# HpWang-whu/RoReg

Hardware: AMD Instinct MI355X
Metric: pair-registrations/sec (higher is better)
Workload: dtype f32 (every f32 operand enters the fp16 matrix cores as hi + lo fp16 under a per-keypoint power-of-two block scale: <= 22 significant bits relative to a CONSERVATIVE per-keypoint bound -- measured on the extractor: the bound sits 2^2..2^6 above the keypoint's true coefficient maximum (config.f16x2_sc

## Files before the change

### roreg_amd/csrc/mfma_match.hip

```cpp
#include "common.h"
#include "primitives.h"

#pragma clang fp contract(off)

namespace {

struct MatchTask {
    const float *desc0, *desc1;
    const int64_t *rows0, *rows1;
    int32_t m0, m1;
};

constexpr int F = 32, TILE = 128, LP = 36;
constexpr float PAD_NORM = 1e30f;

struct WS {
    float *G;
    float *N;
    unsigned *AM;
    unsigned long long *PK;
    unsigned *MX;
};
__host__ __device__ inline size_t ws_task_bytes(int P) { return (size_t)2 * P * (F * 4 + 4 + 4 + 8) + 64; }
__device__ __forceinline__ WS ws_of(char *base, int task, int P) {
    char *p = base + (size_t)task * ws_task_bytes(P);
    WS w;
    w.PK = reinterpret_cast<unsigned long long *>(p); p += (size_t)2 * P * 8;
    w.G = reinterpret_cast<float *>(p); p += (size_t)2 * P * F * 4;
    w.N = reinterpret_cast<float *>(p); p += (size_t)2 * P * 4;
    w.AM = reinterpret_cast<unsigned *>(p); p += (size_t)2 * P * 4;
    w.MX = reinterpret_cast<unsigned *>(p);
    return w;
}

__device__ __forceinline__ unsigned f2o(float x) { const unsigned b = __float_as_uint(x); return b ^ ((b >> 31) ? 0xffffffffu : 0x80000000u); }
__device__ __forceinline__ float o2f(unsigned k) { return __uint_as_float(k ^ ((k >> 31) ? 0x80000000u : 0xffffffffu)); }

__global__ __launch_bounds__(256) void mm_prepare_kernel(const MatchTask *__restrict__ tasks, int P, char *__restrict__ wsb) {
    const int task = blockIdx.z >> 1, side = blockIdx.z & 1;
    const MatchTask t = tasks[task];
    const WS w = ws_of(wsb, task, P);
    const float *desc = side ? t.desc1 : t.desc0;
    const int64_t *rows = side ? t.rows1 : t.rows0;
    const int m = side ? t.m1 : t.m0;
    const int j = blockIdx.x * 8 + (threadIdx.x >> 5), f = threadIdx.x & 31;
    if (blockIdx.x == 0 && threadIdx.x == 0) w.MX[side] = 0u;
    if (j >= P) return;
    float v = 0.f;
    if (j < m) v = desc[(size_t)(rows ? rows[j] : (int64_t)j) * F + f];
    w.G[((size_t)side * P + j) * F + f] = v;
    float s = v * v;
#pragma unroll
    for (int o = 16; o > 0; o >>= 1) s += __shfl_xor(s, o);
    if (f == 0) {
        w.N[(size_t)side * P + j] = j < m ? s : PAD_NORM;
        w.AM[(size_t)side * P + j] = 0xffffffffu;
        w.PK[(size_t)side * P + j] = ~0ull;
    }
}

__global__ __launch_bounds__(256) void mm_maxnorm_kernel(const MatchTask *__restrict__ tasks, int P, char *__restrict__ wsb) {
    const int task = blockIdx.z >> 1, side = blockIdx.z & 1;
    const MatchTask t = tasks[task];
    const WS w = ws_of(wsb, task, P);
    const int m = side ? t.m1 : t.m0;
    const int j = blockIdx.x * 256 + threadIdx.x;
    float v = (j < m) ? w.N[(size_t)side * P + j] : 0.f;
#pragma unroll
    for (int o = 32; o > 0; o >>= 1) v = fmaxf(v, __shfl_xor(v, o));
    if ((threadIdx.x & 63) == 0 && v > 0.f) atomicMax(&w.MX[side], __float_as_uint(v));
}

__device__ __forceinline__ f32x16 mfma6(const bf16x8 (&a)[3], const bf16x8 (&b)[3], f32x16 c) {
    c = __builtin_amdgcn_mfma_f32_32x32x16_bf16(a[2], b[0], c, 0, 0, 0);
    c = __builtin_amdgcn_mfma_f32_32x32x16_bf16(a[1], b[1], c, 0, 0, 0);
    c = __builtin_amdgcn_mfma_f32_32x32x16_bf16(a[0], b[2], c, 0, 0, 0);
    c = __builtin_amdgcn_mfma_f32_32x32x16_bf16(a[1], b[0], c, 0, 0, 0);
    c = __builtin_amdgcn_mfma_f32_32x32x16_bf16(a[0], b[1], c, 0, 0, 0);
    c = __builtin_amdgcn_mfma_f32_32x32x16_bf16(a[0], b[0], c, 0, 0, 0);
    return c;
}

__device__ __forceinline__ int norm_exp(float n2) {
    if (!(n2 > 0.f) || !(n2 < __builtin_inff())) return 0;
    int ex;
    (void)frexpf(n2, &ex);
    return 14 - ((ex + 1) >> 1);
}
__device__ __forceinline__ f32x16 mfma3(const f16x8 (&a)[2], const f16x8 (&b)[2], f32x16 c) {
    c = __builtin_amdgcn_mfma_f32_32x32x16_f16(a[1], b[0], c, 0, 0, 0);
    c = __builtin_amdgcn_mfma_f32_32x32x16_f16(a[0], b[1], c, 0, 0, 0);
    c = __builtin_amdgcn_mfma_f32_32x32x16_f16(a[0], b[0], c, 0, 0, 0);
    return c;
}

__device__ __forceinline__ float exact_dist(const float *__restrict__ s, const float *__restrict__ t) {
    float acc = 0.f;
#pragma unroll
    for (int f = 0; f < F; ++f) {
        const float d = __fsub_rn(s[f], t[f]);
        acc = __fadd_rn(acc, __fmul_rn(d, d));
    }
    return sqrtf(__fadd_rn(acc, 1e-7f));
}

template <bool VERIFY, int NP >
__global__ __launch_bounds__(256, 2) void mm_tile_kernel(const MatchTask *__restrict__ tasks, int P, char *__restrict__ wsb) {
    __shared__ __attribute__((aligned(16))) float S[TILE * LP], T[TILE * LP];
    __shared__ float n0s[TILE], n1s[TILE], thr0[TILE], thr1[TILE];
    __shared__ float xs0[TILE], xs1[TILE], is0[TILE], is1[TILE];
    const int task = blockIdx.z;
    const MatchTask t = tasks[task];
    const int i0 = blockIdx.y * TILE, j0 = blockIdx.x * TILE;
    if (i0 >= t.m0 || j0 >= t.m1) return;
    const WS w = ws_of(wsb, task, P);
    const int tid = threadIdx.x, lane = tid & 63, wv = tid >> 6;
    const int wm = wv & 1, wn = wv >> 1, jl = lane & 31, h = lane >> 5;

    {
        const float4 *g0 = reinterpret_cast<const float4 *>(w.G + (size_t)i0 * F);
        const float4 *g1 = reinterpret_cast<const float4 *>(w.G + ((size_t)P + j0) * F);
        for (int q = tid; q < TILE * F / 4; q += 256) {
            const int r = q >> 3, c4 = q & 7;
            *reinterpret_cast<float4 *>(S + r * LP + c4 * 4) = g0[q];
            *reinterpret_cast<float4 *>(T + r * LP + c4 * 4) = g1[q];
        }
        if (tid < TILE) {
            const float a = w.N[i0 + tid], b = w.N[(size_t)P + j0 + tid];
            n0s[tid] = a; n1s[tid] = b;
            const int ea = NP == 2 ? norm_exp(a) : 0, eb = NP == 2 ? norm_exp(b) : 0;
            xs0[tid] = ldexpf(1.f, ea); is0[tid] = ldexpf(1.f, -ea); xs1[tid] = ldexpf(1.f, eb); is1[tid] = ldexpf(1.f, -eb);
            if (VERIFY) {
                const float mx0 = __uint_as_float(w.MX[0]), mx1 = __uint_as_float(w.MX[1]);
                thr0[tid] = o2f(w.AM[i0 + tid]) + (1e-4f * (a + mx1) + 1e-6f);
                thr1[tid] = o2f(w.AM[(size_t)P + j0 + tid]) + (1e-4f * (b + mx0) + 1e-6f);
            }
        }
    }
    __syncthreads();

    f32x16 c[2][2], ct[2][2];
#pragma unroll
    for (int a = 0; a < 2; ++a)
#pragma unroll
        for (int b = 0; b < 2; ++b)
#pragma unroll
            for (int r = 0; r < 16; ++r) { c[a][b][r] = 0.f; ct[a][b][r] = 0.f; }
#pragma unroll
    for (int st = 0; st < 2; ++st) {
        using frag = typename std::conditional<NP == 3, bf16x8, f16x8>::type;
        frag sf[2][NP], tf[2][NP];
#pragma unroll
        for (int g = 0; g < 2; ++g) {
            float x8[8];
            const int rs = wm * 64 + g * 32 + jl, rt = wn * 64 + g * 32 + jl;
            const float4 *ps = reinterpret_cast<const float4 *>(S + rs * LP + st * 16 + h * 8);
            const float4 u0 = ps[0], u1 = ps[1];
            x8[0] = u0.x; x8[1] = u0.y; x8[2] = u0.z; x8[3] = u0.w; x8[4] = u1.x; x8[5] = u1.y; x8[6] = u1.z; x8[7] = u1.w;
            if constexpr (NP == 3) split3(x8, sf[g][0], sf[g][1], sf[g][2]); else split2(x8, xs0[rs], sf[g][0], sf[g][1]);
            const float4 *pt = reinterpret_cast<const float4 *>(T + rt * LP + st * 16 + h * 8);
            const float4 v0 = pt[0], v1 = pt[1];
            x8[0] = v0.x; x8[1] = v0.y; x8[2] = v0.z; x8[3] = v0.w; x8[4] = v1.x; x8[5] = v1.y; x8[6] = v1.z; x8[7] = v1.w;
            if constexpr (NP == 3) split3(x8, tf[g][0], tf[g][1], tf[g][2]); else split2(x8, xs1[rt], tf[g][0], tf[g][1]);
        }
#pragma unroll
        for (int a = 0; a < 2; ++a)
#pragma unroll
            for (int b = 0; b < 2; ++b) {
                if constexpr (NP == 3) {
                    c[a][b] = mfma6(sf[a], tf[b], c[a][b]);
                    if (!VERIFY) ct[a][b] = mfma6(tf[a], sf[b], ct[a][b]);
                } else {
                    c[a][b] = mfma3(sf[a], tf[b], c[a][b]);
                    if (!VERIFY) ct[a][b] = mfma3(tf[a], sf[b], ct[a][b]);
                }
            }
    }
#define DOT_C(a, b, r, ir, jc) (NP == 2 ? (c[a][b][r] * is0[ir]) * is1[jc] : c[a][b][r])
#define DOT_CT(a, b, r, jr, ic) (NP == 2 ? (ct[a][b][r] * is1[jr]) * is0[ic] : ct[a][b][r])

    if (!VERIFY) {
#pragma unroll
        for (int b = 0; b < 2; ++b) {
            const int jc = wn * 64 + b * 32 + jl;
            const float nj = n1s[jc];
            float mn = __builtin_inff();
#pragma unroll
            for (int a = 0; a < 2; ++a)
#pragma unroll
                for (int r = 0; r < 16; ++r) {
                    const int ir = wm * 64 + a * 32 + (r & 3) + 8 * (r >> 2) + 4 * h;
                    mn = fminf(mn, (n0s[ir] + nj) - 2.f * DOT_C(a, b, r, ir, jc));
                }
            mn = fminf(mn, __shfl_xor(mn, 32));
            if (h == 0 && j0 + jc < t.m1) atomicMin(&w.AM[(size_t)P + j0 + jc], f2o(mn));
        }
#pragma unroll
        for (int b = 0; b < 2; ++b) {
            const int ic = wm * 64 + b * 32 + jl;
            const float ni = n0s[ic];
            float mn = __builtin_inff();
#pragma unroll
            for (int a = 0; a < 2; ++a)
#pragma unroll
                for (int r = 0; r < 16; ++r) {
                    const int jr = wn * 64 + a * 32 + (r & 3) + 8 * (r >> 2) + 4 * h;
                    mn = fminf(mn, (ni + n1s[jr]) - 2.f * DOT_CT(a, b, r, jr, ic));
                }
            mn = fminf(mn, __shfl_xor(mn, 32));
            if (h == 0 && i0 + ic < t.m0) atomicMin(&w.AM[i0 + ic], f2o(mn));
        }
    } else {
#pragma unroll
        for (int b = 0; b < 2; ++b) {
            const int jc = wn * 64 + b * 32 + jl;
            const float nj = n1s[jc], tj = thr1[jc];
#pragma unroll
            for (int a = 0; a < 2; ++a)
#pragma unroll
                for (int r = 0; r < 16; ++r) {
                    const int ir = wm * 64 + a * 32 + (r & 3) + 8 * (r >> 2) + 4 * h;
                    const float av = (n0s[ir] + nj) - 2.f * DOT_C(a, b, r, ir, jc);
                    const bool k0 = av <= thr0[ir], k1 = av <= tj;
                    if (k0 || k1) {
                        const float d = exact_dist(S + ir * LP, T + jc * LP);
                        const unsigned long long db = (unsigned long long)__float_as_uint(d) << 32;
                        if (k0 && j0 + jc < t.m1) atomicMin(&w.PK[i0 + ir], db | (unsigned)(j0 + jc));
                        if (k1 && i0 + ir < t.m0) atomicMin(&w.PK[(size_t)P + j0 + jc], db | (unsigned)(i0 + ir));
                    }
                }
        }
    }
#undef DOT_C
#undef DOT_CT
}

constexpr int TP = TILE * F;
__device__ __forceinline__ int swz_piece(int row, int c) { return row * 8 + (c ^ ((row >> 1) & 7)); }
__device__ __forceinline__ float exact_dist_swz(const float *__restrict__ s_tile, int ir, const float *__restrict__ t_tile, int jc) {
    float acc = 0.f;
#pragma unroll
    for (int f = 0; f < F; ++f) {
        const float sv = s_tile[swz_piece(ir, f >> 2) * 4 + (f & 3)], tv = t_tile[swz_piece(jc, f >> 2) * 4 + (f & 3)];
        const float d = __fsub_rn(sv, tv);
        acc = __fadd_rn(acc, __fmul_rn(d, d));
    }
    return sqrtf(__fadd_rn(acc, 1e-7f));
}

template <bool VERIFY>
__global__ __launch_bounds__(256, 2) void mm_strip_kernel(const MatchTask *__restrict__ tasks, int P, char *__restrict__ wsb) {
    extern __shared__ __attribute__((aligned(16))) char smem[];
    float *S = reinterpret_cast<float *>(smem);
    float *Tb = S + TP;
    float *n0s = Tb + 2 * TP, *xs0 = n0s + TILE, *is0 = xs0 + TILE, *thr0 = is0 + TILE;
    float *n1s = thr0 + TILE, *xs1 = n1s + 2 * TILE, *is1 = xs1 + 2 * TILE, *thr1 = is1 + 2 * TILE;
    unsigned *cm = reinterpret_cast<unsigned *>(thr1 + 2 * TILE);
    const int task = blockIdx.y;
    const MatchTask t = tasks[task];
    const int i0 = blockIdx.x * TILE;
    if (i0 >= t.m0 || t.m1 <= 0) return;
    const WS w = ws_of(wsb, task, P);
    const int tid = threadIdx.x, lane = tid & 63, wv = tid >> 6;
    const int wm = wv & 1, wn = wv >> 1, jl = lane & 31, h = lane >> 5;
    const int ntj = (t.m1 + TILE - 1) / TILE;
    const float mx0 = VERIFY ? __uint_as_float(w.MX[0]) : 0.f, mx1 = VERIFY ? __uint_as_float(w.MX[1]) : 0.f;

    auto dma_tile = [&](const float *src, float *dst) {
#pragma unroll
        for (int k = 0; k < 4; ++k) {
            const int q = k * 256 + tid, row = q >> 3, cs = q & 7;
            __builtin_amdgcn_global_load_lds((const __attribute__((address_space(1))) void *)(src + swz_piece(row, cs) * 4),
                                             (__attribute__((address_space(3))) void *)(dst + (k * 256 + wv * 64) * 4), 16, 0, 0);
        }
    };
    auto load_consts = [&](int jt) -> float {
        const int r = tid & (TILE - 1);
        if (tid < TILE) return w.N[(size_t)P + jt * TILE + r];
        return VERIFY ? o2f(w.AM[(size_t)P + jt * TILE + r]) : 0.f;
    };
    auto store_consts = [&](int buf, float v) {
        const int r = tid & (TILE - 1);
        if (tid < TILE) {
            const int e = norm_exp(v);
            n1s[buf * TILE + r] = v; xs1[buf * TILE + r] = ldexpf(1.f, e); is1[buf * TILE + r] = ldexpf(1.f, -e);
        } else if (VERIFY) thr1[buf * TILE + r] = v;
    };

    dma_tile(w.G + (size_t)i0 * F, S);
    dma_tile(w.G + (size_t)P * F, Tb);
    {
        const float c0 = load_consts(0);
        if (tid < TILE) {
            const float a = w.N[i0 + tid];
            const int e = norm_exp(a);
            n0s[tid] = a; xs0[tid] = ldexpf(1.f, e); is0[tid] = ldexpf(1.f, -e);
            if (VERIFY) thr0[tid] = o2f(w.AM[i0 + tid]) + (1e-4f * (a + mx1) + 1e-6f);
        }
        store_consts(0, c0);
        if (!VERIFY)
            for (int j = tid; j < P; j += 256) cm[j] = 0xffffffffu;
    }
    asm volatile("s_waitcnt vmcnt(0) lgkmcnt(0)" ::: "memory");
    __syncthreads();

    f16x8 sf[2][2][2];
#pragma unroll
    for (int st = 0; st < 2; ++st)
#pragma unroll
        for (int g = 0; g < 2; ++g) {
            const int rs = wm * 64 + g * 32 + jl;
            const float4 u0 = *reinterpret_cast<const float4 *>(S + swz_piece(rs, st * 4 + h * 2) * 4);
            const float4 u1 = *reinterpret_cast<const float4 *>(S + swz_piece(rs, st * 4 + h * 2 + 1) * 4);
            const float x8[8] = {u0.x, u0.y, u0.z, u0.w, u1.x, u1.y, u1.z, u1.w};
            split2(x8, xs0[rs], sf[st][g][0], sf[st][g][1]);
        }
    f32x16 rmin[2];
#pragma unroll
    for (int a = 0; a < 2; ++a)
#pragma unroll
        for (int r = 0; r < 16; ++r) rmin[a][r] = __builtin_inff();

    for (int jt = 0; jt < ntj; ++jt) {
        const int buf = jt & 1, j0 = jt * TILE;
        const float *T = Tb + buf * TP;
        float cnext = 0.f;
        if (jt + 1 < ntj) {
            dma_tile(w.G + ((size_t)P + j0 + TILE) * F, Tb + (buf ^ 1) * TP);
            cnext = load_consts(jt + 1);
        }
        f32x16 c[2][2];
#pragma unroll
        for (int a = 0; a < 2; ++a)
#pragma unroll
            for (int b = 0; b < 2; ++b)
#pragma unroll
                for (int r = 0; r < 16; ++r) c[a][b][r] = 0.f;
#pragma unroll
        for (int st = 0; st < 2; ++st) {
            f16x8 tf[2][2];
#pragma unroll
            for (int g = 0; g < 2; ++g) {
                const int rt = wn * 64 + g * 32 + jl;
                const float4 v0 = *reinterpret_cast<const float4 *>(T + swz_piece(rt, st * 4 + h * 2) * 4);
                const float4 v1 = *reinterpret_cast<const float4 *>(T + swz_piece(rt, st * 4 + h * 2 + 1) * 4);
                const float x8[8] = {v0.x, v0.y, v0.z, v0.w, v1.x, v1.y, v1.z, v1.w};
                split2(x8, xs1[buf * TILE + rt], tf[g][0], tf[g][1]);
            }
#pragma unroll
            for (int a = 0; a < 2; ++a)
#pragma unroll
                for (int b = 0; b < 2; ++b) c[a][b] = mfma3(sf[st][a], tf[b], c[a][b]);
        }
#pragma unroll
        for (int b = 0; b < 2; ++b) {
            const int jc = wn * 64 + b * 32 + jl;
            const float nj = n1s[buf * TILE + jc], isj = is1[buf * TILE + jc];
            if constexpr (!VERIFY) {
                float mn = __builtin_inff();
#pragma unroll
                for (int a = 0; a < 2; ++a)
#pragma unroll
                    for (int r = 0; r < 16; ++r) {
                        const int ir = wm * 64 + a * 32 + (r & 3) + 8 * (r >> 2) + 4 * h;
                        const float av = (n0s[ir] + nj) - 2.f * ((c[a][b][r] * is0[ir]) * isj);
                        mn = fminf(mn, av);
                        rmin[a][r] = fminf(rmin[a][r], av);
                    }
                mn = fminf(mn, __shfl_xor(mn, 32));
                if (h == 0) atomicMin(cm + j0 + jc, f2o(mn));
            } else {
                const float tj = thr1[buf * TILE + jc] + (1e-4f * (nj + mx0) + 1e-6f);
                unsigned m0 = 0u, m1 = 0u;
#pragma unroll
                for (int a = 0; a < 2; ++a)
#pragma unroll
                    for (int r = 0; r < 16; ++r) {
                        const int ir = wm * 64 + a * 32 + (r & 3) + 8 * (r >> 2) + 4 * h;
                        const float av = (n0s[ir] + nj) - 2.f * ((c[a][b][r] * is0[ir]) * isj);
                        m0 |= (av <= thr0[ir] ? 1u : 0u) << (a * 16 + r);
                        m1 |= (av <= tj ? 1u : 0u) << (a * 16 + r);
                    }
                unsigned m = m0 | m1;
                while (m) {
                    const int q = __ffs(m) - 1;
                    m &= m - 1;
                    const int ir = wm * 64 + (q >> 4) * 32 + (q & 3) + 8 * ((q & 15) >> 2) + 4 * h;
                    const float d = exact_dist_swz(S, ir, T, jc);
                    const unsigned long long db = (unsigned long long)__float_as_uint(d) << 32;
                    if (((m0 >> q) & 1u) && j0 + jc < t.m1) atomicMin(&w.PK[i0 + ir], db | (unsigned)(j0 + jc));
                    if (((m1 >> q) & 1u) && i0 + ir < t.m0) atomicMin(&w.PK[(size_t)P + j0 + jc], db | (unsigned)(i0 + ir));
                }
            }
        }
        if (jt + 1 < ntj) store_consts(buf ^ 1, cnext);
        asm volatile("s_waitcnt vmcnt(0) lgkmcnt(0)" ::: "memory");
        __syncthreads();
    }
    if constexpr (!VERIFY) {
#pragma unroll
        for (int a = 0; a < 2; ++a)
#pragma unroll
            for (int r = 0; r < 16; ++r) {
                float v = rmin[a][r];
#pragma unroll
                for (int o = 16; o > 0; o >>= 1) v = fminf(v, __shfl_xor(v, o));
                const int ir = wm * 64 + a * 32 + (r & 3) + 8 * (r >> 2) + 4 * h;
                if (jl == 0 && i0 + ir < t.m0) atomicMin(&w.AM[i0 + ir], f2o(v));
            }
        for (int j = tid; j < t.m1; j += 256) atomicMin(&w.AM[(size_t)P + j], cm[j]);
    }
}

__global__ __launch_bounds__(1024) void mm_mutual_kernel(const MatchTask *__restrict__ tasks, int P, char *__restrict__ wsb, int out_pitch,
                                                         int64_t *__restrict__ match_all, int32_t *__restrict__ counts) {
    __shared__ int wave_cnt[16];
    __shared__ int base;
    const int task = blockIdx.x;
    const MatchTask t = tasks[task];
    const WS w = ws_of(wsb, task, P);
    const unsigned long long *p01 = w.PK, *p10 = w.PK + P;
    int64_t *match_out = match_all + (size_t)task * out_pitch * 2;
    const int m = t.m1 > 0 ? t.m0 : 0;
    const int tid = threadIdx.x, lane = tid & 63, wv = tid >> 6;
    if (tid == 0) base = 0;
    __syncthreads();
    for (int start = 0; start < m; start += 1024) {
        const int i = start + tid;
        bool keep = false;
        int64_t j = 0;
        if (i < m) {
            j = (int64_t)(p01[i] & 0xffffffffu);
            keep = j < (int64_t)t.m1 && (int64_t)(p10[j] & 0xffffffffu) == (int64_t)i;
        }
        const unsigned long long mask = __ballot(keep);
        const int before = __popcll(mask & ((1ull << lane) - 1ull));
        if (lane == 0) wave_cnt[wv] = __popcll(mask);
        __syncthreads();
        int woff = 0, total = 0;
#pragma unroll
        for (int q = 0; q < 16; ++q) {
            const int cq = wave_cnt[q];
            if (q < wv) woff += cq;
            total += cq;
        }
        const int b0 = base;
        if (keep) {
            const int pos = b0 + woff + before;
            match_out[2 * pos] = t.rows0 ? t.rows0[i] : (int64_t)i;
            match_out[2 * pos + 1] = t.rows1 ? t.rows1[j] : j;
        }
        __syncthreads();
        if (tid == 0) base = b0 + total;
        __syncthreads();
    }
    if (tid == 0) counts[task] = base;
}

}

extern "C" size_t roreg_mutual_match_batch_workspace(int n_tasks, int max_m) {
    const int P = (max_m + TILE - 1) / TILE * TILE;
    return (size_t)n_tasks * ws_task_bytes(P > 0 ? P : TILE);
}

extern "C" int roreg_mutual_match_batch(const roreg_match_task *tasks_dev, int n_tasks, int max_m, int64_t *match_out, int32_t *counts_out,
                                        void *workspace, size_t workspace_bytes, void *stream) {
    if (n_tasks == 0) return 0;
    ROREG_REQUIRE(tasks_dev && match_out && counts_out && workspace && n_tasks > 0 && max_m >= 0, "roreg_mutual_match_batch: bad arguments");
    ROREG_REQUIRE(workspace_bytes >= roreg_mutual_match_batch_workspace(n_tasks, max_m), "roreg_mutual_match_batch: workspace too small");
    ROREG_REQUIRE(n_tasks <= 65535, "roreg_mutual_match_batch: too many tasks in one call (%d)", n_tasks);
    static_assert(sizeof(roreg_match_task) == sizeof(MatchTask), "roreg_match_task layout");
    hipStream_t s = roreg::as_stream(stream);
    const MatchTask *tasks = reinterpret_cast<const MatchTask *>(tasks_dev);
    const int P = max_m > 0 ? (max_m + TILE - 1) / TILE * TILE : TILE;
    char *ws = reinterpret_cast<char *>(workspace);
    const int out_pitch = (max_m + 1) & ~1;
    if (max_m > 0) {
        hipLaunchKernelGGL(mm_prepare_kernel, dim3(P / 8, 1, 2 * n_tasks), dim3(256), 0, s, tasks, P, ws);
        hipLaunchKernelGGL(mm_maxnorm_kernel, dim3(P / 256 + 1, 1, 2 * n_tasks), dim3(256), 0, s, tasks, P, ws);
        const dim3 grid(P / TILE, P / TILE, n_tasks);
        roreg::ProfScope prof(roreg::PROF_MM_TILE, s);
        static const bool bf16x3 = [] { const char *e = getenv("ROREG_MATCH_BF16X3"); return e && e[0] == '1'; }();
        static const bool tiles = [] { const char *e = getenv("ROREG_MATCH_TILES"); return e && e[0] == '1'; }();
        const size_t lds_strip = (size_t)(3 * TP + 12 * TILE) * 4 + (size_t)P * 4;
        if (!bf16x3 && !tiles && lds_strip <= 80 * 1024) {
            const dim3 sgrid(P / TILE, n_tasks);
            auto ka = mm_strip_kernel<false>; auto kb = mm_strip_kernel<true>;
            hipError_t e1 = hipFuncSetAttribute(reinterpret_cast<const void *>(ka), hipFuncAttributeMaxDynamicSharedMemorySize, (int)lds_strip);
            hipError_t e2 = hipFuncSetAttribute(reinterpret_cast<const void *>(kb), hipFuncAttributeMaxDynamicSharedMemorySize, (int)lds_strip);
            if (e1 != hipSuccess || e2 != hipSuccess) { roreg::set_error("roreg_mutual_match_batch: hipFuncSetAttribute(%zu) failed", lds_strip); return 1; }
            hipLaunchKernelGGL(ka, sgrid, dim3(256), lds_strip, s, tasks, P, ws);
            hipLaunchKernelGGL(kb, sgrid, dim3(256), lds_strip, s, tasks, P, ws);
        } else if (bf16x3) {
            hipLaunchKernelGGL((mm_tile_kernel<false, 3>), grid, dim3(256), 0, s, tasks, P, ws);
            hipLaunchKernelGGL((mm_tile_kernel<true, 3>), grid, dim3(256), 0, s, tasks, P, ws);
        } else {
            hipLaunchKernelGGL((mm_tile_kernel<false, 2>), grid, dim3(256), 0, s, tasks, P, ws);
            hipLaunchKernelGGL((mm_tile_kernel<true, 2>), grid, dim3(256), 0, s, tasks, P, ws);
        }
    }
    hipLaunchKernelGGL(mm_mutual_kernel, dim3(n_tasks), dim3(1024), 0, s, tasks, P, ws, out_pitch, match_out, counts_out);
    ROREG_CHECK_LAUNCH("roreg_mutual_match_batch");
    return 0;
}
```

Before: 1063.

## Precompute fp16 hi/lo splits, triple-buffer tiles, queue exact-distance checks in LDS

The prepare kernel now computes the scaled fp16 hi/lo split of each descriptor once and stores it in a new workspace buffer. The strip kernel DMAs these fp16 tiles straight into a three-slot LDS ring, prefetching two tiles ahead with a partial vmcnt wait. This removes the per-tile split work and the per-tile norm-constant setup. In the verify pass, candidate pairs are pushed into an LDS queue and the exact distances are computed later from global fp32 rows, instead of immediately from the swizzled LDS tiles. That evens out warp divergence but adds workspace memory, global reads during the drain, and more complex synchronisation.

```diff
diff --git a/roreg_amd/csrc/mfma_match.hip b/roreg_amd/csrc/mfma_match.hip
--- a/roreg_amd/csrc/mfma_match.hip
+++ b/roreg_amd/csrc/mfma_match.hip
@@ -16,17 +16,19 @@
 
 struct WS {
     float *G;
+    _Float16 *H;
     float *N;
     unsigned *AM;
     unsigned long long *PK;
     unsigned *MX;
 };
-__host__ __device__ inline size_t ws_task_bytes(int P) { return (size_t)2 * P * (F * 4 + 4 + 4 + 8) + 64; }
+__host__ __device__ inline size_t ws_task_bytes(int P) { return (size_t)2 * P * (F * 4 + F * 4 + 4 + 4 + 8) + 64; }
 __device__ __forceinline__ WS ws_of(char *base, int task, int P) {
     char *p = base + (size_t)task * ws_task_bytes(P);
     WS w;
     w.PK = reinterpret_cast<unsigned long long *>(p); p += (size_t)2 * P * 8;
     w.G = reinterpret_cast<float *>(p); p += (size_t)2 * P * F * 4;
+    w.H = reinterpret_cast<_Float16 *>(p); p += (size_t)2 * P * F * 4;
     w.N = reinterpret_cast<float *>(p); p += (size_t)2 * P * 4;
     w.AM = reinterpret_cast<unsigned *>(p); p += (size_t)2 * P * 4;
     w.MX = reinterpret_cast<unsigned *>(p);
@@ -35,6 +37,13 @@
 
 __device__ __forceinline__ unsigned f2o(float x) { const unsigned b = __float_as_uint(x); return b ^ ((b >> 31) ? 0xffffffffu : 0x80000000u); }
 __device__ __forceinline__ float o2f(unsigned k) { return __uint_as_float(k ^ ((k >> 31) ? 0x80000000u : 0xffffffffu)); }
+
+__device__ __forceinline__ int norm_exp(float n2) {
+    if (!(n2 > 0.f) || !(n2 < __builtin_inff())) return 0;
+    int ex;
+    (void)frexpf(n2, &ex);
+    return 14 - ((ex + 1) >> 1);
+}
 
 __global__ __launch_bounds__(256) void mm_prepare_kernel(const MatchTask *__restrict__ tasks, int P, char *__restrict__ wsb) {
     const int task = blockIdx.z >> 1, side = blockIdx.z & 1;
@@ -52,8 +61,19 @@
     float s = v * v;
 #pragma unroll
     for (int o = 16; o > 0; o >>= 1) s += __shfl_xor(s, o);
+    const float nrm = j < m ? s : PAD_NORM;
+    float x8[8];
+#pragma unroll
+    for (int e = 0; e < 8; ++e) x8[e] = __shfl(v, (f & 3) * 8 + e, 32);
+    if (f < 4) {
+        f16x8 hi, lo;
+        split2(x8, ldexpf(1.f, norm_exp(nrm)), hi, lo);
+        _Float16 *hrow = w.H + ((size_t)side * P + j) * (2 * F);
+        *reinterpret_cast<f16x8 *>(hrow + f * 8) = hi;
+        *reinterpret_cast<f16x8 *>(hrow + F + f * 8) = lo;
+    }
     if (f == 0) {
-        w.N[(size_t)side * P + j] = j < m ? s : PAD_NORM;
+        w.N[(size_t)side * P + j] = nrm;
         w.AM[(size_t)side * P + j] = 0xffffffffu;
         w.PK[(size_t)side * P + j] = ~0ull;
     }
@@ -81,12 +101,6 @@
     return c;
 }
 
-__device__ __forceinline__ int norm_exp(float n2) {
-    if (!(n2 > 0.f) || !(n2 < __builtin_inff())) return 0;
-    int ex;
-    (void)frexpf(n2, &ex);
-    return 14 - ((ex + 1) >> 1);
-}
 __device__ __forceinline__ f32x16 mfma3(const f16x8 (&a)[2], const f16x8 (&b)[2], f32x16 c) {
     c = __builtin_amdgcn_mfma_f32_32x32x16_f16(a[1], b[0], c, 0, 0, 0);
     c = __builtin_amdgcn_mfma_f32_32x32x16_f16(a[0], b[1], c, 0, 0, 0);
@@ -237,70 +251,96 @@
 
 constexpr int TP = TILE * F;
 __device__ __forceinline__ int swz_piece(int row, int c) { return row * 8 + (c ^ ((row >> 1) & 7)); }
-__device__ __forceinline__ float exact_dist_swz(const float *__restrict__ s_tile, int ir, const float *__restrict__ t_tile, int jc) {
+
+__device__ __forceinline__ unsigned lds_addr(const void *p) { return (unsigned)(size_t)(const __attribute__((address_space(3))) void *)p; }
+__device__ __forceinline__ void lds_umin(unsigned addr, unsigned v) { asm volatile("ds_min_u32 %0, %1" ::"v"(addr), "v"(v) : "memory"); }
+__device__ __forceinline__ void lds_store(unsigned addr, unsigned v) { asm volatile("ds_write_b32 %0, %1" ::"v"(addr), "v"(v) : "memory"); }
+__device__ __forceinline__ unsigned lds_add_rtn(unsigned addr, unsigned v) {
+    unsigned r;
+    asm volatile("ds_add_rtn_u32 %0, %1, %2\n\ts_waitcnt lgkmcnt(0)" : "=v"(r) : "v"(addr), "v"(v) : "memory");
+    return r;
+}
+
+__device__ __forceinline__ void exact_update(const WS &w, const MatchTask &t, int P, int i, int j, bool k0, bool k1) {
+    const float4 *ps = reinterpret_cast<const float4 *>(w.G + (size_t)i * F);
+    const float4 *pt = reinterpret_cast<const float4 *>(w.G + ((size_t)P + j) * F);
     float acc = 0.f;
 #pragma unroll
-    for (int f = 0; f < F; ++f) {
-        const float sv = s_tile[swz_piece(ir, f >> 2) * 4 + (f & 3)], tv = t_tile[swz_piece(jc, f >> 2) * 4 + (f & 3)];
-        const float d = __fsub_rn(sv, tv);
-        acc = __fadd_rn(acc, __fmul_rn(d, d));
-    }
-    return sqrtf(__fadd_rn(acc, 1e-7f));
+    for (int q0 = 0; q0 < F / 4; q0 += 2) {
+        const float4 u[2] = {ps[q0], ps[q0 + 1]}, v[2] = {pt[q0], pt[q0 + 1]};
+#pragma unroll
+        for (int q = 0; q < 2; ++q) {
+            const float sv[4] = {u[q].x, u[q].y, u[q].z, u[q].w}, tv[4] = {v[q].x, v[q].y, v[q].z, v[q].w};
+#pragma unroll
+            for (int f = 0; f < 4; ++f) {
+                const float d = __fsub_rn(sv[f], tv[f]);
+                acc = __fadd_rn(acc, __fmul_rn(d, d));
+            }
+        }
+    }
+    const float d = sqrtf(__fadd_rn(acc, 1e-7f));
+    const unsigned long long db = (unsigned long long)__float_as_uint(d) << 32;
+    if (k0 && j < t.m1) atomicMin(&w.PK[i], db | (unsigned)j);
+    if (k1 && i < t.m0) atomicMin(&w.PK[(size_t)P + j], db | (unsigned)i);
 }
 
 template <bool VERIFY>
 __global__ __launch_bounds__(256, 2) void mm_strip_kernel(const MatchTask *__restrict__ tasks, int P, char *__restrict__ wsb) {
     extern __shared__ __attribute__((aligned(16))) char smem[];
-    float *S = reinterpret_cast<float *>(smem);
-    float *Tb = S + TP;
-    float *n0s = Tb + 2 * TP, *xs0 = n0s + TILE, *is0 = xs0 + TILE, *thr0 = is0 + TILE;
-    float *n1s = thr0 + TILE, *xs1 = n1s + 2 * TILE, *is1 = xs1 + 2 * TILE, *thr1 = is1 + 2 * TILE;
-    unsigned *cm = reinterpret_cast<unsigned *>(thr1 + 2 * TILE);
+    char *ring = smem;
+    float *n0s = reinterpret_cast<float *>(ring + 3 * TP * 4), *k0s = n0s + TILE, *thr0 = k0s + TILE;
+    float *n1s = thr0 + TILE;
+    unsigned *am1 = reinterpret_cast<unsigned *>(n1s + 3 * TILE);
+    unsigned *cm = am1 + 3 * TILE;
+    unsigned *qctl = cm;
+    unsigned *queue = cm + 4;
+    const unsigned QCAP = (unsigned)P + 3 * TILE - 4;
     const int task = blockIdx.y;
     const MatchTask t = tasks[task];
     const int i0 = blockIdx.x * TILE;
     if (i0 >= t.m0 || t.m1 <= 0) return;
     const WS w = ws_of(wsb, task, P);
-    const int tid = threadIdx.x, lane = tid & 63, wv = tid >> 6;
+    const int tid = threadIdx.x, lane = tid & 63, wv = __builtin_amdgcn_readfirstlane(tid >> 6);
     const int wm = wv & 1, wn = wv >> 1, jl = lane & 31, h = lane >> 5;
     const int ntj = (t.m1 + TILE - 1) / TILE;
     const float mx0 = VERIFY ? __uint_as_float(w.MX[0]) : 0.f, mx1 = VERIFY ? __uint_as_float(w.MX[1]) : 0.f;
-
-    auto dma_tile = [&](const float *src, float *dst) {
-#pragma unroll
-        for (int k = 0; k < 4; ++k) {
-            const int q = k * 256 + tid, row = q >> 3, cs = q & 7;
-            __builtin_amdgcn_global_load_lds((const __attribute__((address_space(1))) void *)(src + swz_piece(row, cs) * 4),
-                                             (__attribute__((address_space(3))) void *)(dst + (k * 256 + wv * 64) * 4), 16, 0, 0);
-        }
+    const char *H0 = reinterpret_cast<const char *>(w.H), *H1 = H0 + (size_t)P * (4 * F);
+
+    const unsigned piece0 = (unsigned)swz_piece(tid >> 3, tid & 7) * 16u;
+    auto dma_rows = [&](const char *src, char *dst) {
+#pragma unroll
+        for (int k = 0; k < 4; ++k)
+            __builtin_amdgcn_global_load_lds((const __attribute__((address_space(1))) void *)(src + k * 4096 + (size_t)piece0),
+                                             (__attribute__((address_space(3))) void *)(dst + (k * 256 + wv * 64) * 16), 16, 0, 0);
     };
-    auto load_consts = [&](int jt) -> float {
-        const int r = tid & (TILE - 1);
-        if (tid < TILE) return w.N[(size_t)P + jt * TILE + r];
-        return VERIFY ? o2f(w.AM[(size_t)P + jt * TILE + r]) : 0.f;
+    const char *csrc = (VERIFY && wv >= 2) ? reinterpret_cast<const char *>(w.AM + (size_t)P) : reinterpret_cast<const char *>(w.N + (size_t)P);
+    const unsigned word0 = (unsigned)(tid & (TILE - 1)) * 4u;
+    auto dma_tile = [&](int jt) {
+        const int slot = jt % 3;
+        dma_rows(H1 + (size_t)jt * TILE * (4 * F), ring + slot * (TP * 4));
+        char *dst = reinterpret_cast<char *>(n1s) + ((wv >> 1) * 3 * TILE + slot * TILE + (wv & 1) * 64) * 4;
+        __builtin_amdgcn_global_load_lds((const __attribute__((address_space(1))) void *)(csrc + (size_t)jt * TILE * 4 + (size_t)word0),
+                                         (__attribute__((address_space(3))) void *)dst, 4, 0, 0);
     };
-    auto store_consts = [&](int buf, float v) {
-        const int r = tid & (TILE - 1);
-        if (tid < TILE) {
-            const int e = norm_exp(v);
-            n1s[buf * TILE + r] = v; xs1[buf * TILE + r] = ldexpf(1.f, e); is1[buf * TILE + r] = ldexpf(1.f, -e);
-        } else if (VERIFY) thr1[buf * TILE + r] = v;
+    auto drain = [&]() {
+        const unsigned n = min(qctl[0], QCAP);
+        for (unsigned k = tid; k < n; k += 256) {
+            const unsigned e = queue[k];
+            exact_update(w, t, P, i0 + (int)(e & 127u), (int)((e >> 7) & 8191u), (e >> 20) & 1u, (e >> 21) & 1u);
+        }
     };
 
-    dma_tile(w.G + (size_t)i0 * F, S);
-    dma_tile(w.G + (size_t)P * F, Tb);
-    {
-        const float c0 = load_consts(0);
-        if (tid < TILE) {
-            const float a = w.N[i0 + tid];
-            const int e = norm_exp(a);
-            n0s[tid] = a; xs0[tid] = ldexpf(1.f, e); is0[tid] = ldexpf(1.f, -e);
-            if (VERIFY) thr0[tid] = o2f(w.AM[i0 + tid]) + (1e-4f * (a + mx1) + 1e-6f);
-        }
-        store_consts(0, c0);
-        if (!VERIFY)
-            for (int j = tid; j < P; j += 256) cm[j] = 0xffffffffu;
-    }
+    dma_rows(H0 + (size_t)i0 * (4 * F), ring + 2 * (TP * 4));
+    dma_tile(0);
+    if (ntj > 1) dma_tile(1);
+    if (tid < TILE) {
+        const float a = w.N[i0 + tid];
+        n0s[tid] = a; k0s[tid] = -2.f * ldexpf(1.f, -norm_exp(a));
+        if (VERIFY) thr0[tid] = o2f(w.AM[i0 + tid]) + (1e-4f * (a + mx1) + 1e-6f);
+    }
+    if constexpr (!VERIFY) {
+        for (int j = tid; j < P; j += 256) cm[j] = 0xffffffffu;
+    } else if (tid < 3) qctl[tid] = 0u;
     asm volatile("s_waitcnt vmcnt(0) lgkmcnt(0)" ::: "memory");
     __syncthreads();
 
@@ -308,27 +348,29 @@
 #pragma unroll
     for (int st = 0; st < 2; ++st)
 #pragma unroll
-        for (int g = 0; g < 2; ++g) {
-            const int rs = wm * 64 + g * 32 + jl;
-            const float4 u0 = *reinterpret_cast<const float4 *>(S + swz_piece(rs, st * 4 + h * 2) * 4);
-            const float4 u1 = *reinterpret_cast<const float4 *>(S + swz_piece(rs, st * 4 + h * 2 + 1) * 4);
-            const float x8[8] = {u0.x, u0.y, u0.z, u0.w, u1.x, u1.y, u1.z, u1.w};
-            split2(x8, xs0[rs], sf[st][g][0], sf[st][g][1]);
-        }
+        for (int g = 0; g < 2; ++g)
+#pragma unroll
+            for (int p = 0; p < 2; ++p)
+                sf[st][g][p] = *reinterpret_cast<const f16x8 *>(ring + 2 * (TP * 4) + swz_piece(wm * 64 + g * 32 + jl, p * 4 + st * 2 + h) * 16);
+    float n0r[2][16], k0r[2][16], t0r[2][16];
     f32x16 rmin[2];
 #pragma unroll
     for (int a = 0; a < 2; ++a)
 #pragma unroll
-        for (int r = 0; r < 16; ++r) rmin[a][r] = __builtin_inff();
+        for (int r = 0; r < 16; ++r) {
+            const int ir = wm * 64 + a * 32 + (r & 3) + 8 * (r >> 2) + 4 * h;
+            n0r[a][r] = n0s[ir]; k0r[a][r] = k0s[ir];
+            t0r[a][r] = VERIFY ? thr0[ir] : 0.f;
+            rmin[a][r] = __builtin_inff();
+        }
+
+    asm volatile("s_waitcnt lgkmcnt(0)" ::: "memory");
+    __syncthreads();
 
     for (int jt = 0; jt < ntj; ++jt) {
-        const int buf = jt & 1, j0 = jt * TILE;
-        const float *T = Tb + buf * TP;
-        float cnext = 0.f;
-        if (jt + 1 < ntj) {
-            dma_tile(w.G + ((size_t)P + j0 + TILE) * F, Tb + (buf ^ 1) * TP);
-            cnext = load_consts(jt + 1);
-        }
+        const int slot = jt % 3, j0 = jt * TILE;
+        const char *T = ring + slot * (TP * 4);
+        if (jt + 2 < ntj) dma_tile(jt + 2);
         f32x16 c[2][2];
 #pragma unroll
         for (int a = 0; a < 2; ++a)
@@ -340,62 +382,90 @@
         for (int st = 0; st < 2; ++st) {
             f16x8 tf[2][2];
 #pragma unroll
-            for (int g = 0; g < 2; ++g) {
-                const int rt = wn * 64 + g * 32 + jl;
-                const float4 v0 = *reinterpret_cast<const float4 *>(T + swz_piece(rt, st * 4 + h * 2) * 4);
-                const float4 v1 = *reinterpret_cast<const float4 *>(T + swz_piece(rt, st * 4 + h * 2 + 1) * 4);
-                const float x8[8] = {v0.x, v0.y, v0.z, v0.w, v1.x, v1.y, v1.z, v1.w};
-                split2(x8, xs1[buf * TILE + rt], tf[g][0], tf[g][1]);
-            }
+            for (int g = 0; g < 2; ++g)
+#pragma unroll
+                for (int p = 0; p < 2; ++p)
+                    tf[g][p] = *reinterpret_cast<const f16x8 *>(T + swz_piece(wn * 64 + g * 32 + jl, p * 4 + st * 2 + h) * 16);
 #pragma unroll
             for (int a = 0; a < 2; ++a)
 #pragma unroll
                 for (int b = 0; b < 2; ++b) c[a][b] = mfma3(sf[st][a], tf[b], c[a][b]);
         }
-#pragma unroll
-        for (int b = 0; b < 2; ++b) {
-            const int jc = wn * 64 + b * 32 + jl;
-            const float nj = n1s[buf * TILE + jc], isj = is1[buf * TILE + jc];
-            if constexpr (!VERIFY) {
-                float mn = __builtin_inff();
+        float nj[2], isj[2];
+#pragma unroll
+        for (int b = 0; b < 2; ++b) { nj[b] = n1s[slot * TILE + wn * 64 + b * 32 + jl]; isj[b] = ldexpf(1.f, -norm_exp(nj[b])); }
+#define MM_AV(a, b, r) __fmaf_rn(c[a][b][r] * k0r[a][r], isj[b], n0r[a][r] + nj[b])
+        if constexpr (!VERIFY) {
+            float mn[2] = {__builtin_inff(), __builtin_inff()};
+#pragma unroll
+            for (int a = 0; a < 2; ++a)
+#pragma unroll
+                for (int r = 0; r < 16; r += 2) {
+                    const float a00 = MM_AV(a, 0, r), a01 = MM_AV(a, 0, r + 1), a10 = MM_AV(a, 1, r), a11 = MM_AV(a, 1, r + 1);
+                    mn[0] = fminf(mn[0], fminf(a00, a01)); mn[1] = fminf(mn[1], fminf(a10, a11));
+                    rmin[a][r] = fminf(rmin[a][r], fminf(a00, a10)); rmin[a][r + 1] = fminf(rmin[a][r + 1], fminf(a01, a11));
+                }
+#pragma unroll
+            for (int b = 0; b < 2; ++b) {
+                const float v = fminf(mn[b], __shfl_xor(mn[b], 32));
+                if (h == 0) lds_umin(lds_addr(cm + j0 + wn * 64 + b * 32 + jl), f2o(v));
+            }
+        } else {
+#pragma unroll
+            for (int b = 0; b < 2; ++b) {
+                const int jc = wn * 64 + b * 32 + jl;
+                const float tj = o2f(am1[slot * TILE + jc]) + (1e-4f * (nj[b] + mx0) + 1e-6f);
+                unsigned m0 = 0u, m1 = 0u;
+                unsigned long long any = 0ull;
 #pragma unroll
                 for (int a = 0; a < 2; ++a)
 #pragma unroll
-                    for (int r = 0; r < 16; ++r) {
-                        const int ir = wm * 64 + a * 32 + (r & 3) + 8 * (r >> 2) + 4 * h;
-                        const float av = (n0s[ir] + nj) - 2.f * ((c[a][b][r] * is0[ir]) * isj);
-                        mn = fminf(mn, av);
-                        rmin[a][r] = fminf(rmin[a][r], av);
+                    for (int rg = 0; rg < 16; rg += 4) {
+                        float av[4];
+                        unsigned long long hit = 0ull;
+#pragma unroll
+                        for (int q = 0; q < 4; ++q) {
+                            av[q] = MM_AV(a, b, rg + q);
+                            hit |= __ballot(av[q] <= t0r[a][rg + q]) | __ballot(av[q] <= tj);
+                        }
+                        if (hit) {
+#pragma unroll
+                            for (int q = 0; q < 4; ++q) {
+                                m0 |= (av[q] <= t0r[a][rg + q] ? 1u : 0u) << (a * 16 + rg + q);
+                                m1 |= (av[q] <= tj ? 1u : 0u) << (a * 16 + rg + q);
+                            }
+                            any |= hit;
+                        }
                     }
-                mn = fminf(mn, __shfl_xor(mn, 32));
-                if (h == 0) atomicMin(cm + j0 + jc, f2o(mn));
-            } else {
-                const float tj = thr1[buf * TILE + jc] + (1e-4f * (nj + mx0) + 1e-6f);
-                unsigned m0 = 0u, m1 = 0u;
-#pragma unroll
-                for (int a = 0; a < 2; ++a)
-#pragma unroll
-                    for (int r = 0; r < 16; ++r) {
-                        const int ir = wm * 64 + a * 32 + (r & 3) + 8 * (r >> 2) + 4 * h;
-                        const float av = (n0s[ir] + nj) - 2.f * ((c[a][b][r] * is0[ir]) * isj);
-                        m0 |= (av <= thr0[ir] ? 1u : 0u) << (a * 16 + r);
-                        m1 |= (av <= tj ? 1u : 0u) << (a * 16 + r);
+                if (any) {
+                    unsigned m = m0 | m1;
+                    while (m) {
+                        const int q = __ffs(m) - 1;
+                        m &= m - 1;
+                        const int ir = wm * 64 + (q >> 4) * 32 + (q & 3) + 8 * ((q & 15) >> 2) + 4 * h;
+                        const unsigned k0 = (m0 >> q) & 1u, k1 = (m1 >> q) & 1u;
+                        const unsigned slot = lds_add_rtn(lds_addr(qctl), 1u);
+                        if (slot < QCAP) lds_store(lds_addr(queue + slot), (unsigned)ir | ((unsigned)(j0 + jc) << 7) | (k0 << 20) | (k1 << 21));
+                        else exact_update(w, t, P, i0 + ir, j0 + jc, k0, k1);
                     }
-                unsigned m = m0 | m1;
-                while (m) {
-                    const int q = __ffs(m) - 1;
-                    m &= m - 1;
-                    const int ir = wm * 64 + (q >> 4) * 32 + (q & 3) + 8 * ((q & 15) >> 2) + 4 * h;
-                    const float d = exact_dist_swz(S, ir, T, jc);
-                    const unsigned long long db = (unsigned long long)__float_as_uint(d) << 32;
-                    if (((m0 >> q) & 1u) && j0 + jc < t.m1) atomicMin(&w.PK[i0 + ir], db | (unsigned)(j0 + jc));
-                    if (((m1 >> q) & 1u) && i0 + ir < t.m0) atomicMin(&w.PK[(size_t)P + j0 + jc], db | (unsigned)(i0 + ir));
                 }
             }
         }
-        if (jt + 1 < ntj) store_consts(buf ^ 1, cnext);
-        asm volatile("s_waitcnt vmcnt(0) lgkmcnt(0)" ::: "memory");
-        __syncthreads();
+#undef MM_AV
+        if (jt + 2 < ntj) asm volatile("s_waitcnt vmcnt(5) lgkmcnt(0)" ::: "memory");
+        else asm volatile("s_waitcnt vmcnt(0) lgkmcnt(0)" ::: "memory");
+        __builtin_amdgcn_s_barrier();
+        asm volatile("" ::: "memory");
+        if constexpr (VERIFY) {
+            const unsigned seen = qctl[1 + ((jt + 1) & 1)];
+            if (tid == 0) lds_store(lds_addr(qctl + 1 + (jt & 1)), qctl[0]);
+            if (seen > QCAP / 2) {
+                drain();
+                __syncthreads();
+                if (tid < 3) qctl[tid] = 0u;
+                __syncthreads();
+            }
+        }
     }
     if constexpr (!VERIFY) {
 #pragma unroll
@@ -409,6 +479,8 @@
                 if (jl == 0 && i0 + ir < t.m0) atomicMin(&w.AM[i0 + ir], f2o(v));
             }
         for (int j = tid; j < t.m1; j += 256) atomicMin(&w.AM[(size_t)P + j], cm[j]);
+    } else {
+        drain();
     }
 }
 
```

After: 1072 (median of 6 runs). Within noise of the previous version (+0.9%).
